# biomedia-mira/causal-gen

Hardware: AMD Instinct MI355X
Metric: HVAE train images/sec (higher is better)
Workload: dtype f16; 1 GPU; ukbb192 HVAE train step (192x192x1, DGauss likelihood, beta=5.0, z_max_res=96); per_gpu_batch=32, global_batch=32, parallelism=dp1, hipgraph=True, params=17371122

## Files before the change

causal-gen_amd/_lib.py:

```python
import ctypes as C
import os

_HERE = os.path.dirname(os.path.abspath(__file__))
LIB_PATH = os.environ.get("CGEN_LIB") or os.path.join(_HERE, "libcgen_hip.so")

F32, F16, F32S = 0, 1, 2
DMOL_LOW_BIT = 0x100
ACT_NONE, ACT_RELU, ACT_GELU = 0, 1, 2
UNARY_LEAKY_RELU, UNARY_CLAMP_MIN, UNARY_ADD = 3, 4, 5
MAX_SEG = 4


class View(C.Structure):
    _fields_ = [("p", C.c_void_p), ("sn", C.c_int64), ("sh", C.c_int64), ("sw", C.c_int64), ("c", C.c_int32),
                ("cpad", C.c_int32)]


NULL_VIEW = View(None, 0, 0, 0, 0, 0)


class ConvArgs(C.Structure):
    _fields_ = [("dtype", C.c_int32), ("n", C.c_int32), ("h", C.c_int32), ("w", C.c_int32), ("ks", C.c_int32),
                ("nseg", C.c_int32), ("act", C.c_int32), ("dact", C.c_int32), ("seg", View * MAX_SEG),
                ("weight", C.c_void_p), ("bias", C.c_void_p), ("out", View), ("aux", View), ("res1", View), ("res2", View),
                ("out_rem", C.c_int64), ("res1_rem", C.c_int64)]


class Block3Out(C.Structure):
    _fields_ = [("w", C.c_void_p), ("bias", C.c_void_p), ("out", View), ("aux", View), ("res1", View),
                ("out_rem", C.c_int64), ("res1_rem", C.c_int64)]


class Block3Args(C.Structure):
    _fields_ = [("dtype", C.c_int32), ("n", C.c_int32), ("h", C.c_int32), ("w", C.c_int32), ("nseg", C.c_int32),
                ("nout", C.c_int32), ("pre_act", C.c_int32), ("reserved", C.c_int32), ("seg", View * MAX_SEG),
                ("w_a", C.c_void_p), ("bias_a", C.c_void_p), ("mid", View), ("mid_aux", View), ("o", Block3Out * 2), ("w_a16", C.c_void_p)]


class Block4Args(C.Structure):
    _fields_ = [("dtype", C.c_int32), ("n", C.c_int32), ("h", C.c_int32), ("w", C.c_int32), ("nseg", C.c_int32),
                ("nout", C.c_int32), ("fwd", C.c_int32), ("b", C.c_int32), ("seg", View * MAX_SEG),
                ("wimg", C.c_void_p * 3), ("bias", C.c_void_p * 3), ("mid", View * 3), ("mid_aux", View * 3), ("o", Block3Out * 3)]


class WgradArgs(C.Structure):
    _fields_ = [("dtype", C.c_int32), ("n", C.c_int32), ("h", C.c_int32), ("w", C.c_int32), ("ks", C.c_int32),
                ("nseg", C.c_int32), ("act", C.c_int32), ("nsplit", C.c_int32), ("seg", View * MAX_SEG), ("gout", View),
                ("partial_w", C.c_void_p), ("partial_b", C.c_void_p)]


class WprepDesc(C.Structure):
# ... 267 lines not shown
```

causal-gen_amd/csrc/block.hip:

```cpp
#include <stddef.h>
#include <stdlib.h>

#include <algorithm>
#include <type_traits>

#include "common.h"

namespace cgen {

typedef float f32x16 __attribute__((ext_vector_type(16)));
typedef short s16x2v __attribute__((ext_vector_type(2)));

__device__ uint4 g_b3zero[4];

#define B3_TW 16
#define B3_HW 20
#define B3_MW 18
#define B3_XS 80
constexpr int b3_ndi(int th) { return ((th + 4) * B3_HW + 47) / 48; }
constexpr int b3_xbytes(int th) { return 4 * b3_ndi(th) * 12 * B3_XS + 64; }
constexpr int b3_nmp(int th) { return (th + 2) * B3_MW; }

struct BV3 { const char* p; int sn, sh, sw; };
struct B3Out {
// ... 5 lines not shown
};
struct B3P {
  int N, H, W, nseg, nch, b, nout, nksB;
  int tiles_x, tiles_y, ntiles, ctot8;
  int ns, wb_persist, scratch_off, bias_off;
  int tm_off, tm_bytes, pad1, pad2;
  Div32 d_tx, d_ty;
  BV3 seg[3];
  int seg_koff[4];
  int seg_c8[3];
  int small, s_rows, s_strips, s_nmb;
  int s_mid_off, s_kt_off, s_red_off, s_dbg, s_segk0[3], s_segg[3];
  Div32 s_dg1, s_dxw, s_dw, s_dstrips, s_dnb;
  int rows, r_rs, r_sx, r_sy, r_res_tile, r_pad;
  const char* wA16;
  const char* wA;
  const float* biasA;
  BV3 mid, mid_aux;
  B3Out o[2];
  unsigned long long* stamps;
};

__device__ __forceinline__ void b3_pin(h16x8& v) { asm volatile("" : "+v"(v)); }
__device__ __forceinline__ h16x8 b3_relu8(h16x8 v) {
  union { h16x8 h; s16x2v s[4]; } c;
  c.h = v;
#pragma unroll
  for (int e = 0; e < 4; ++e) c.s[e] = __builtin_elementwise_max(c.s[e], (s16x2v){0, 0});
  return c.h;
}
// ... 933 lines not shown
  constexpr size_t off_b = (sizeof(B3P) + alignof(B3P) - 1) / alignof(B3P) * alignof(B3P);
  const int koff = second ? (int)off_b : 0;
  typedef const B3P __attribute__((address_space(4)))* kp_ptr;
  const B3P& p = *(const B3P*)(kp_ptr)((const char __attribute__((address_space(4)))*)__builtin_amdgcn_kernarg_segment_ptr() + koff);
  blk3s_body<false>(p, second ? (int)blockIdx.x - na : (int)blockIdx.x, second ? (int)gridDim.x - na : na, koff);
}

#define B3R_NW 8
#define B3R_XC 36
#define B3R_MC 34
#define B3R_NG 4
#define B3R_MR 16
constexpr int b3r_grpb(int nch) { return ((4 * B3R_XC * (nch * 4 + 1) * 16 + 1023) / 1024) * 1024; }
constexpr int b3r_mrowb(int nb) { return B3R_MC * ((nb & 1) ? nb : nb + 1) * 16; }
constexpr size_t b3r_lds(int nch, int nb) { return (size_t)B3R_NG * b3r_grpb(nch) + (size_t)B3R_MR * b3r_mrowb(nb) + 1024; }

template <bool PRE, int NCH, int NB, int RES>
__global__ __launch_bounds__(64 * B3R_NW, 2) void blk3r_kernel(B3P p) {
  __builtin_amdgcn_s_setprio(3);
  constexpr int G1 = NCH * 4 + 1, XS = G1 * 16, ROWB = B3R_XC * XS, GRPB = b3r_grpb(NCH), NINST = GRPB / 1024, IPW = (NINST + B3R_NW - 1) / B3R_NW;
  constexpr int NBS = (NB & 1) ? NB : NB + 1, MS = NBS * 16, MROWB = B3R_MC * MS;
  constexpr int KA = 9 * NCH, NKB = (9 * NB + 1) / 2;
  constexpr bool AUX = !PRE;
  typedef __attribute__((address_space(3))) void* lds_ptr;
  extern __shared__ __attribute__((aligned(16))) char smem[];
  char* const X = smem;
  char* const MID = smem + B3R_NG * GRPB;
  char* const SCR = MID + B3R_MR * MROWB;
  const char* const zero = (const char*)g_b3zero;
  const int tid = threadIdx.x, lane = tid & 63, wave = __builtin_amdgcn_readfirstlane(tid >> 6);
  const int H = p.H, W = p.W, bch = p.b;
  const int item = blockIdx.x;
  const int sx = item % p.r_sx, t1 = item / p.r_sx, sy = t1 % p.r_sy, n = t1 / p.r_sy;
  const int x0 = sx * 32, Y0 = sy * p.r_rs, Yend = min(Y0 + p.r_rs, H), nbands = (Yend - Y0 + 3) >> 2;
  const BV3 sv = p.seg[0];
  const char* const xin = sv.p + n * sv.sn;
  auto dma_group = [&](const int gi) {
    const uint32_t gbase = (uint32_t)(uintptr_t)(lds_ptr)(X + (gi & (B3R_NG - 1)) * GRPB);
    const uint32_t sbase = (uint32_t)(uintptr_t)(lds_ptr)SCR;
    const int row0 = Y0 - 2 + 4 * gi;
#pragma unroll
    for (int t = 0; t < IPW; ++t) {
      const int ii = wave + B3R_NW * t;
      const int sl = ii * 64 + lane;
      const int r = sl / (B3R_XC * G1), rem = sl - r * (B3R_XC * G1), px = rem / G1, g = rem - px * G1;
      const int iy = row0 + r, ix = x0 - 2 + px;
      const bool ok = ii < NINST && r < 4 && (unsigned)iy < (unsigned)H && (unsigned)ix < (unsigned)W && g < G1 - 1;
      const char* src = ok ? xin + iy * sv.sh + ix * sv.sw + g * 16 : zero;
      b3_dma16(src, ii < NINST ? gbase + ii * 1024 : sbase);
    }
  };
  dma_group(0);
  dma_group(1);
  dma_group(2);
  h16x8 Aw[KA], Bw[NKB];
  {
    const char* wa = p.wA16 + lane * 16;
#pragma unroll
    for (int s_ = 0; s_ < KA; ++s_) Aw[s_] = *(const h16x8*)(wa + s_ * 1024);
    const int pair_w = min(wave >> 2, p.o[0].npb - 1);
    const char* wb = p.o[0].w + (size_t)pair_w * NKB * 1024 + lane * 16;
#pragma unroll
    for (int i = 0; i < NKB; ++i) Bw[i] = *(const h16x8*)(wb + i * 1024);
  }
  const int l16 = lane & 15, l4 = lane >> 4;
  int pr[2], pc[2];
#pragma unroll
  for (int j = 0; j < 2; ++j) {
    const int q = min(16 * (wave + B3R_NW * j) + l16, 4 * B3R_MC - 1);
    pr[j] = q / B3R_MC; pc[j] = q - pr[j] * B3R_MC;
  }
  const int chA = 4 * l4;
  float biasA[4] = {0.f, 0.f, 0.f, 0.f};
  if constexpr (PRE) {
    if (p.biasA != nullptr && chA < bch) { const float4 b4 = *(const float4*)(p.biasA + chA); biasA[0] = b4.x; biasA[1] = b4.y; biasA[2] = b4.z; biasA[3] = b4.w; }
  }
  const B3Out& O = p.o[0];
  const int npb = O.npb, Co = O.Co;
  const int pairB = wave >> 2, rB = wave & 3;
  const bool jobB = pairB < npb;
  const int pxB = lane & 31, kgB = lane >> 5;
  const int ch0 = pairB * 32 + 16 * kgB;
  int koff[NKB], kty[NKB];
#pragma unroll
  for (int i = 0; i < NKB; ++i) {
    const int u = 2 * i + kgB, tp = min(u / NB, 8), gq = u - (u / NB) * NB;
    kty[i] = tp / 3;
    koff[i] = (pxB + tp % 3) * MS + gq * 16;
  }
  float biasB[16];
#pragma unroll
  for (int e = 0; e < 16; ++e) biasB[e] = 0.f;
  if (jobB && O.bias != nullptr) {
#pragma unroll
    for (int e = 0; e < 16; e += 4)
      if (ch0 + e < Co) { const float4 b4 = *(const float4*)(O.bias + ch0 + e); biasB[e] = b4.x; biasB[e + 1] = b4.y; biasB[e + 2] = b4.z; biasB[e + 3] = b4.w; }
  }
  B3_VMWAIT();
#pragma unroll
  for (int s_ = 0; s_ < KA; ++s_) b3_pin(Aw[s_]);
#pragma unroll
  for (int i = 0; i < NKB; ++i) b3_pin(Bw[i]);
#pragma unroll
  for (int e = 0; e < 4; ++e) asm volatile("" : "+v"(biasA[e]));
#pragma unroll
  for (int e = 0; e < 16; ++e) asm volatile("" : "+v"(biasB[e]));
  B3_BARRIER();

  b3_u32x2 tm[2];
  b3_u32x4 ea[2], er[2];
  tm[0] = tm[1] = (b3_u32x2){0u, 0u};
  ea[0] = ea[1] = er[0] = er[1] = (b3_u32x4){0u, 0u, 0u, 0u};
  auto band_loads = [&](const int m0, const int nrow, const int y) {
    if constexpr (!PRE) {
#pragma unroll
      for (int j = 0; j < 2; ++j) {
        const int m = m0 + pr[j], col = x0 - 1 + pc[j];
        const bool ok = 16 * (wave + B3R_NW * j) + l16 < nrow * B3R_MC && (unsigned)m < (unsigned)H && (unsigned)col < (unsigned)W && chA < bch;
        b3_gload_v8(tm[j], ok ? p.mid_aux.p + (n * p.mid_aux.sn + m * p.mid_aux.sh + col * p.mid_aux.sw) + chA * 2 : zero);
      }
    }
// ... 56 lines not shown
        r.s[0] = __builtin_elementwise_max(r.s[0], (s16x2v){0, 0});
        r.s[1] = __builtin_elementwise_max(r.s[1], (s16x2v){0, 0});
        ol = r.u;
      } else {
        v[0] = h_lo(tm[j].x) > 0.f ? v[0] : 0.f; v[1] = h_hi(tm[j].x) > 0.f ? v[1] : 0.f;
        v[2] = h_lo(tm[j].y) > 0.f ? v[2] : 0.f; v[3] = h_hi(tm[j].y) > 0.f ? v[3] : 0.f;
        o.x = f2h_pk(v[0], v[1]); o.y = f2h_pk(v[2], v[3]);
        ol = o;
      }
      if (own) *(uint2*)((char*)p.mid.p + (n * p.mid.sn + m * p.mid.sh + col * p.mid.sw) + chA * 2) = o;
      *(uint2*)(MID + (m & (B3R_MR - 1)) * MROWB + pc[j] * MS + chA * 2) = in_img ? ol : make_uint2(0, 0);
    }
  };
  band_loads(Y0 - 1, 2, -1);
  phaseA(Y0 - 1, 2, 0);
  for (int k = 0; k < nbands; ++k) {
    const int Y = Y0 + 4 * k, y = Y + rB;
    B3_BARRIER();
    band_loads(Y + 1, 4, y);
    dma_group(k + 3);
    phaseA(Y + 1, 4, 1);
    B3_BARRIER();
    if (jobB) {
      const int ox = x0 + pxB;
      const bool ev = y < Yend && ox < W;
      int rowb[3];
#pragma unroll
      for (int ty = 0; ty < 3; ++ty) rowb[ty] = ((y - 1 + ty) & (B3R_MR - 1)) * MROWB;
      f32x16 c;
#pragma unroll
      for (int e = 0; e < 16; ++e) c[e] = biasB[e];
#pragma unroll
      for (int i = 0; i < NKB; ++i) {
        const int rb = kty[i] == 0 ? rowb[0] : (kty[i] == 1 ? rowb[1] : rowb[2]);
        const h16x8 bq = *(const h16x8*)(MID + rb + koff[i]);
        c = b3_mfma(Bw[i], bq, c);
      }
      if constexpr (RES == 1) {
        const int rel = y - (Y0 - 2);
        const char* rp = X + ((rel >> 2) & (B3R_NG - 1)) * GRPB + (rel & 3) * ROWB + (pxB + 2) * XS + (ch0 >> 3) * 16;
        er[0] = *(const b3_u32x4*)rp;
        er[1] = *(const b3_u32x4*)(rp + 16);
      }
#pragma unroll
      for (int q8 = 0; q8 < 2; ++q8) {
        if (!(ev && ch0 + 8 * q8 < Co)) continue;
        float u[8];
#pragma unroll
        for (int e = 0; e < 8; ++e) u[e] = c[8 * q8 + e];
        if constexpr (AUX) {
          const uint32_t w[4] = {ea[q8].x, ea[q8].y, ea[q8].z, ea[q8].w};
#pragma unroll
          for (int e = 0; e < 4; ++e) {
            u[2 * e] = h_lo(w[e]) > 0.f ? u[2 * e] : 0.f;
            u[2 * e + 1] = h_hi(w[e]) > 0.f ? u[2 * e + 1] : 0.f;
          }
        }
        if constexpr (RES != 0) {
          const uint32_t w[4] = {er[q8].x, er[q8].y, er[q8].z, er[q8].w};
#pragma unroll
          for (int e = 0; e < 4; ++e) { u[2 * e] += h_lo(w[e]); u[2 * e + 1] += h_hi(w[e]); }
        }
        *(uint4*)((char*)O.out.p + (n * O.out.sn + y * O.out.sh + ox * O.out.sw) + ch0 * 2 + 16 * q8) = b3_pack8(u);
      }
    }
  }
  B3_VMWAIT();
}

static bool b3_view(const cgen_view& v, int n, int h, int w, BV3& o) {
  o.p = (const char*)v.p; o.sn = o.sh = o.sw = 0;
  if (!v.p) return true;
  const int64_t ext = ((int64_t)n * v.sn + (int64_t)(h + 12 + 4) * v.sh + (int64_t)(w + B3_TW + 4) * v.sw + v.c + 64) * 2;
  if (ext >= ((int64_t)1 << 31) || v.sn < 0 || v.sh < 0 || v.sw < 0) return false;
  if (((uintptr_t)v.p % 16) || (v.sn * 2) % 16 || (v.sh * 2) % 16 || (v.sw * 2) % 16) return false;
  o.sn = (int)(v.sn * 2); o.sh = (int)(v.sh * 2); o.sw = (int)(v.sw * 2);
  return true;
}
// ... 40 lines not shown
    if (s.out_rem < 0 || s.res1_rem < 0 || s.out_rem >= ((int64_t)1 << 31) || s.res1_rem >= ((int64_t)1 << 31) || (s.out_rem % 16) || (s.res1_rem % 16)) return 0;
    if ((s.out_rem || s.res1_rem) && (!a->pre_act || a->nout != 1)) return 0;
    if (s.res1_rem && !s.res1.p) return 0;
    d.out_rem = (int)s.out_rem; d.res_rem = (int)s.res1_rem;
    if (!b3_view(s.out, a->n, a->h, a->w, d.out) || !b3_view(s.aux, a->n, a->h, a->w, d.aux) || !b3_view(s.res1, a->n, a->h, a->w, d.res)) return 0;
    if ((s.aux.p && s.aux.c != s.out.c) || (s.res1.p && s.res1.c != s.out.c)) return 0;
    if (o == 0 && s.out.c > 224 && !p.small) return 0;
    if (o > 0 && s.bias) return 0;
  }
  {
    static const int rows_on = [] { const char* e = getenv("CGEN_BLK3R"); return e ? atoi(e) : 1; }();
    const int c0 = a->seg[0].c, co0 = a->o[0].out.c;
    p.rows = (rows_on && !p.small && a->w_a16 && a->nseg == 1 && a->nout == 1 && (c0 == 32 || c0 == 64) && (p.b == 8 || p.b == 16)
              && (co0 == 32 || co0 == 64) && a->w >= 48 && a->h >= 16 && !a->o[0].out_rem && !a->o[0].res1_rem
              && ((uintptr_t)a->w_a16 % 16) == 0) ? 1 : 0;
    if (p.rows) {
      p.wA16 = (const char*)a->w_a16;
      p.r_sx = ceil_div(p.W, 32);
      const int slots = 256;
      long best = -1;
      for (int rs = 8; rs < p.H + 4; rs += 4) {
        const int rsc = rs > p.H ? ((p.H + 3) & ~3) : rs;
        const long wgs = (long)p.N * p.r_sx * ceil_div(p.H, rsc), cost = (long)ceil_div(wgs, slots) * (rsc + 16);
        if (best < 0 || cost < best) { best = cost; p.r_rs = rsc; }
      }
      { static const int rs_env = [] { const char* e = getenv("CGEN_BLK3R_RS"); return e ? atoi(e) : 0; }(); if (rs_env >= 4) p.r_rs = std::min((rs_env + 3) & ~3, (p.H + 3) & ~3); }
      p.r_sy = ceil_div(p.H, p.r_rs);
      p.ntiles = p.N * p.r_sx * p.r_sy;
      const cgen_view& rv = a->o[0].res1;
      p.r_res_tile = (a->pre_act && rv.p && rv.p == a->seg[0].p && rv.sn == a->seg[0].sn && rv.sh == a->seg[0].sh && rv.sw == a->seg[0].sw && co0 == c0) ? 1 : 0;
// ... 131 lines not shown
  if (pa.rows || pb.rows) return 0;
  if (pa.small || pb.small) {
    La.grid = pa.ntiles; Lb.grid = pb.ntiles;
    La.lds = b3s_lds(pa); Lb.lds = b3s_lds(pb);
    La.npg = Lb.npg = 0; La.sm = Lb.sm = 0; La.th = Lb.th = 0;
    return (pa.small && pb.small && !pa.o[0].out_rem && !pb.o[0].out_rem) ? 1 : 0;
  }
  const int ta = pa.ntiles, tb = pb.ntiles;
  La = b3_plan(pa, tb);
  Lb = b3_plan(pb, ta);
  if (La.sm || Lb.sm || La.npg != Lb.npg || La.th != Lb.th || pa.b != pb.b) return 0;
  if (pa.o[0].out_rem || pa.o[0].res_rem || pb.o[0].out_rem || pb.o[0].res_rem) return 0;
  return 1;
}

}

using namespace cgen;

extern "C" int cgen_block3_pair_supported(const cgen_block3_args* a, const cgen_block3_args* b) {
  B3P pa, pb;
  B3Launch La, Lb;
  return b3_pair_plan(a, b, pa, pb, La, Lb);
}

extern "C" int cgen_block3_pair(const cgen_block3_args* a, const cgen_block3_args* b, cgen_stream_t stream) {
  B3P pa, pb;
  B3Launch La, Lb;
  CGEN_REQUIRE(b3_pair_plan(a, b, pa, pb, La, Lb), "cgen_block3_pair: the two problems do not plan to the same data-gradient instance (ask cgen_block3_pair_supported first)");
  if (pa.small) {
// ... 11 lines not shown
  if (trace) fprintf(stderr, "blk3 pair[bwd] %dx%dx%d b %d | grids %d + %d, lds %zu, tile rows %d\n", a->n, a->h, a->w, pa.b, La.grid, Lb.grid, std::max(La.lds, Lb.lds), La.th);
  return check_launch("cgen_block3_pair");
}

extern "C" int cgen_block3_supported(const cgen_block3_args* a) {
  B3P p;
  return b3_fill(a, p);
}

extern "C" int cgen_block3(const cgen_block3_args* a, cgen_stream_t stream) {
  B3P p;
  CGEN_REQUIRE(b3_fill(a, p), "cgen_block3: shape / layout not served by the fused Block kernel (ask cgen_block3_supported first)");
  CGEN_REQUIRE((a->pre_act != 0) == (a->mid_aux.p == nullptr), "cgen_block3: pre_act = 1 is the forward pass (no mid_aux), pre_act = 0 the data gradient (mid_aux = the forward mid)");
  if (p.rows) {
    const int nch = a->seg[0].c / 32, nb = p.b / 8;
    const size_t lds = b3r_lds(nch, nb);
#define B3R_LAUNCH(PRE_, NCH_, NB_, RES_) do { (void)hipFuncSetAttribute((const void*)blk3r_kernel<PRE_, NCH_, NB_, RES_>, hipFuncAttributeMaxDynamicSharedMemorySize, 160 * 1024); \
    hipLaunchKernelGGL((blk3r_kernel<PRE_, NCH_, NB_, RES_>), dim3(p.ntiles), dim3(64 * B3R_NW), lds, (hipStream_t)stream, p); } while (0)
#define B3R_RES(PRE_, NCH_, NB_) do { if (res_mode == 0) B3R_LAUNCH(PRE_, NCH_, NB_, 0); else if (res_mode == 1) B3R_LAUNCH(PRE_, NCH_, NB_, 1); else B3R_LAUNCH(PRE_, NCH_, NB_, 2); } while (0)
#define B3R_RES_BWD(NCH_, NB_) do { if (res_mode == 0) B3R_LAUNCH(false, NCH_, NB_, 0); else B3R_LAUNCH(false, NCH_, NB_, 2); } while (0)
    const int res_mode = !a->o[0].res1.p ? 0 : (p.r_res_tile ? 1 : 2);
    if (a->pre_act) { if (nch == 1) { if (nb == 1) B3R_RES(true, 1, 1); else B3R_RES(true, 1, 2); } else { if (nb == 1) B3R_RES(true, 2, 1); else B3R_RES(true, 2, 2); } }
    else { if (nch == 1) { if (nb == 1) B3R_RES_BWD(1, 1); else B3R_RES_BWD(1, 2); } else { if (nb == 1) B3R_RES_BWD(2, 1); else B3R_RES_BWD(2, 2); } }
#undef B3R_RES
#undef B3R_RES_BWD
#undef B3R_LAUNCH
    static const bool trace_r = getenv("CGEN_CONV_TRACE") != nullptr;
    if (trace_r) fprintf(stderr, "blk3r[%s] %dx%dx%d c %d b %d Co %d | strips %d x %d of %d rows, grid %d, lds %zu, residual from the tile %d\n", a->mid_aux.p ? "bwd" : "fwd", a->n, a->h, a->w,
                         a->seg[0].c, p.b, p.o[0].Co, p.r_sx, p.r_sy, p.r_rs, p.ntiles, lds, p.r_res_tile);
    return check_launch("cgen_block3(rows)");
  }
  if (p.small) {
    const size_t lds = b3s_lds(p);
    if (a->pre_act) {
      (void)hipFuncSetAttribute((const void*)blk3s_kernel<true>, hipFuncAttributeMaxDynamicSharedMemorySize, 160 * 1024);
      hipLaunchKernelGGL((blk3s_kernel<true>), dim3(p.ntiles), dim3(64 * B3S_NW), lds, (hipStream_t)stream, p);
    } else {
      (void)hipFuncSetAttribute((const void*)blk3s_kernel<false>, hipFuncAttributeMaxDynamicSharedMemorySize, 160 * 1024);
// ... 14 lines not shown
```

causal-gen_amd/engine.py:

```python
import ctypes as C
import os
import math

import torch

from . import _lib
from .pairing import BlockRec, PairSlot, may_pair
from .wgrad_sched import WgradMixin
from ._lib import ACT_GELU, ACT_NONE, ACT_RELU, F16, F32, F32S, NULL_VIEW, UNARY_CLAMP_MIN, UNARY_LEAKY_RELU, View

_ALIGN = 256


def _ceil(a, m):
    return (a + m - 1) // m * m


def compact_parents(t):
    if t.dim() == 2:
        return t
    if t.dim() == 4 and ((t.shape[2] == 1 and t.shape[3] == 1) or (t.stride(2) == 0 and t.stride(3) == 0)):
        return t[:, :, 0, 0]
    return None

# ... 251 lines not shown
        self._wg_deferred = []
        self.fwd_branch = os.environ.get("CGEN_FWD_BRANCH", "1") != "0"
        self.infer_branch = os.environ.get("CGEN_INFER_BRANCH", "1") != "0"
        self.fwd_mainfirst = os.environ.get("CGEN_FWD_MAINFIRST", "1") != "0"
        self._fwd_side = None
        self._side_join_pending = False
        self.blk3_on = int(os.environ.get("CGEN_BLK3", "2")) if self.dt == F16 else 0
        self.blk3_minres = int(os.environ.get("CGEN_BLK3_MINRES", "16"))
        self.blk3_small = int(os.environ.get("CGEN_BLK3S", "1"))
        self.blk4_on = int(os.environ.get("CGEN_BLK4", "1")) if self.dt == F16 else 0
        self.blk4_launches = 0
        self.blk4_pair = os.environ.get("CGEN_BLK4_PAIR", "1") != "0"
        self._blk4 = PairSlot(self, self._block4_single, self._block4_pair,
                              lambda h, a: self.lib.block4_pair_supported(C.byref(h), C.byref(a)))
        self.blk3_rows = int(os.environ.get("CGEN_BLK3R", "1"))
        self.blk3_res = self._side_ranges(os.environ.get("CGEN_BLK3_RES", "20-64"))
        self.blk3_res3 = self._side_ranges(os.environ.get("CGEN_BLK3_RES3", "20-112"))
        self.split_frac = float(os.environ.get("CGEN_DP_SPLIT_FRAC", "0.8"))
        self.on_split = None
        self.early_final = None

    blk3_pairs = property(lambda self: self._blk3.pairs, lambda self, v: setattr(self._blk3, "pairs", v))
    blk4_pairs = property(lambda self: self._blk4.pairs, lambda self, v: setattr(self._blk4, "pairs", v))
    conv_pairs = property(lambda self: self._conv.pairs, lambda self, v: setattr(self._conv, "pairs", v))

    @property
    def trunk_rem(self):
        return self.dt != F32 and (self.trunk_mode >= 2 or (self.trunk_mode == 1 and not self.recording))

    def set_loss_scale(self, n_terms):
# ... 301 lines not shown
                self._dbg_names[id(out.base)] = site.name
            (self.tape if tape_hold is None else tape_hold).append((self._bw_conv, (site, segs, act, out, res1, res2), self._bw_tag))
        return out

    @staticmethod
    def _side_ranges(spec):
        out = []
        for v in spec.split(","):
            v = v.strip()
            if not v or v == "0":
                continue
            lo, _, hi = v.partition("-")
            out.append((int(lo), int(hi or lo)))
        return out

    def block2(self, site1, site2, segs, act, res1=None, trunk=False):
        x0 = segs[0]
        res_ok = self.blk3_res3 if len(segs) >= 3 else self.blk3_res
        small = self.blk3_small and x0.w <= 14 and x0.h <= 64 and min(x0.h, x0.w) >= 4
        tile_ok = (min(x0.h, x0.w) >= self.blk3_minres and site1.co <= 32
                   and (not res_ok or any(lo <= x0.h <= hi for lo, hi in res_ok)))
        rows = (self.blk3_rows and len(segs) == 1 and "a16_fwd" in site1.frag and "a16_dg" in site2.frag and x0.w >= 48 and x0.h >= 16
                and not (trunk and self.trunk_rem))
        if (self.blk3_on and act == ACT_RELU and "a_fwd" in site1.frag and "b_fwd" in site2.frag and len(segs) <= 3
                and site1.co % 8 == 0 and site2.co % 8 == 0
                and ((small and site1.co <= 64) or tile_ok or rows)):
            out = self._block3_fwd(site1, site2, segs, res1, trunk, need_rows=rows and not tile_ok and not small)
            if out is not None:
                return out
        t = self.conv(site1, segs, act)
        return self.conv(site2, [t], act, res1=res1, trunk=trunk)

# ... 16 lines not shown
        sup = self.lib.block3_supported(C.byref(a))
        if not sup or (need_rows and sup != 2):
            return None
        if not self._ablated(x0):
            self._timed("conv_fwd", (site1, site2), x0, lambda: self.lib.block3(C.byref(a), self.stream))
        if self.recording:
            if self._dbg_names is not None:
                self._dbg_names[id(out.base)] = site2.name
            if self.blk3_on >= 2:
                self.tape.append((self._bw_block3, BlockRec((site1, site2), segs, (t,), out, res1), self._bw_tag))
            else:
                self.tape.append((self._bw_conv, (site1, segs, ACT_RELU, t, None, None), self._bw_tag))
                self.tape.append((self._bw_conv, (site2, [t], ACT_RELU, out, res1, None), self._bw_tag))
        return out

    def _ablated(self, x0, site=None, tag=None):
        ab = self._ablate
        if not ab:
            return False
        if site is not None and ((tag in ab and site.name.endswith({"f1": ".conv.1", "d3": ".conv.3"}[tag])) or ("r12" in ab and x0.h <= 12)):
            return True
        return any(x0.h == r and ("r%d" % r) in ab for r in (24, 48, 96, 192))

    def _block3_dgrad_args(self, site1, site2, g, gmid, t, outs):
        a = _lib.Block3Args()
        a.dtype, a.n, a.h, a.w, a.nseg, a.nout, a.pre_act = self.dt, g.n, g.h, g.w, 1, len(outs), 0
        a.seg[0] = g.cv()
        a.w_a, a.bias_a = site2.frag["a_dg"], None
        a.w_a16 = site2.frag.get("a16_dg") if self.blk3_rows else None
        a.mid, a.mid_aux = gmid.cv(), t.cv()
        for j, (k, gv, sg, prev) in enumerate(outs):
            a.o[j].w, a.o[j].bias = site1.frag[("b_dg", k)], None
            a.o[j].out, a.o[j].aux = gv.cv(), sg.cv()
            a.o[j].res1 = prev.cv() if prev is not None else NULL_VIEW
        return a

    def _bw_block3(self, sites, segs, mids, out, res1):
        (site1, site2), (t,) = sites, mids
        g = self.grad_read(out)
        if g is None:
            self._blk3.flush()
            return
        act = ACT_RELU
        dsegs = [k for k, sg in enumerate(segs) if sg.rg and site1.seg_rg[k]]
        ok = (1 <= len(dsegs) <= 2 and "a_dg" in site2.frag and all(("b_dg", k) in site1.frag for k in dsegs)
              and all(segs[k].c % 8 == 0 for k in dsegs) and g.c % 8 == 0)
        if ok:
            probe = self._block3_dgrad_args(site1, site2, g, t, t, [(k, segs[k], segs[k], None) for k in dsegs])
            ok = bool(self.lib.block3_supported(C.byref(probe)))
        if not ok:
            self._blk3.flush()
            self._bw_conv(site2, [t], act, out, res1, None)
            self._bw_conv(site1, segs, act, t, None, None)
            return
        if res1 is not None and res1.rg:
            self._blk3.flush()
            self._grad_residual(res1, g, out, [t])
        if self._needs_wgrad(site2) and "wg" not in self._ablate:
            self._wgrad(site2, [t], act, g)
        gt, acc_t = self.grad_write(t)
        assert not acc_t
        tgt = [(k,) + self._dgrad_target(segs[k]) for k in dsegs]
        a = self._block3_dgrad_args(site1, site2, g, gt, t, [(k, gv, segs[k], prev if acc else None) for (k, gv, prev, acc) in tgt])
        x0 = segs[0]
        late = (lambda: self._wgrad(site1, segs, act, gt)) if (self._needs_wgrad(site1) and "wg" not in self._ablate) else (lambda: None)
        if self._ablated(x0):
            self._blk3.flush()
        elif self.lib.block3_supported(C.byref(a)):
            wr = {id(gt.base)} | {id(gv.base) for (_, gv, _, _) in tgt}
            rd = {id(g.base), id(t.base)} | {id(segs[k].base) for (k, _, _, _) in tgt} | {id(prev.base) for (_, _, prev, acc) in tgt if acc}
            self._blk3.submit(a, wr, rd, (sites, x0), late)
            return
        else:
            self._blk3.flush()
            self._dgrad_launch(site2, g, t, 0, act, t, gt, gt, False)
            for (k, gv, prev, acc) in tgt:
                self._dgrad_launch(site1, gt, segs[k], k, act, x0, gv, prev, acc)
        late()

    def _block3_single(self, a, info):
        sites, x0 = info
        self._timed("conv_dgrad", sites, x0, lambda: self.lib.block3(C.byref(a), self.stream))

    def block4(self, sites, segs, res1=None, trunk=False):
        s0, s1, s2, s3 = sites
# ... 550 lines not shown
            self._wg_total = sum(2.0 * st.ci * st.taps * st.co * x0.n * x0.h * x0.w
                                 for fn, a, _ in self.tape for st, x0 in self._entry_sites(fn, a) if self._needs_wgrad(st))
        main_t = torch.cuda.current_stream(self.device)
        if self._side_join_pending:
            self.join_side()
        self.blk3_pairs = self.conv_pairs = self.blk4_pairs = self.lat_tails = 0
        skip = 0
        tape = self.tape
        for i in range(len(tape) - 1, -1, -1):
            fn, args, _ = tape[i]
            if fn == self._bw_block3 or fn == self._bw_block4:
                slot, other, on = (self._blk3, self._blk4, self.blk3_pair) if fn == self._bw_block3 else (self._blk4, self._blk3, self.blk4_pair)
                other.flush()
                if on and slot.held is None and may_pair(tape[i], tape[i - 1] if i > 0 else None):
                    slot.arm()
                fn(*args)
                slot.disarm()
            else:
                self._blk3.flush()
                self._blk4.flush()
                if skip:
                    skip -= 1
                    continue
                if self.lat_tail and fn == self._bw_conv and self.dt == F16 and self.prof is None:
                    ents = self._latent_tail_at(i)
                    if ents is not None and self._bw_latent_tail(*ents):
                        skip = (2 if ents[0] is not None else 1)
                        continue
                if self.conv_pair and fn == self._bw_conv and self.dt != F32 and self._two_unfused_blocks(i):
                    self._conv.arm()
                    fn(*args)
# ... 259 lines not shown
```

causal-gen_amd/vae.py:

```python
import math
import os
from typing import Dict, List, Optional

import numpy as np
import weakref

import torch
from torch import Tensor, nn

from . import _lib
from ._lib import ACT_GELU, ACT_NONE, ACT_RELU, NULL_VIEW
from .engine import ConvSite, Engine

EPS = -9


def _flat_f32(name, *ts):
    lib = _lib.load()
    _lib.require_gpu()
    out = []
    shape, dev = ts[0].shape, ts[0].device
    for t in ts:
        if not (isinstance(t, torch.Tensor) and t.is_cuda and t.device == dev and t.shape == shape):
            raise _lib.CgenError(f"{name}: expects same-shaped tensors on one GPU (there is no CPU path)")
# ... 67 lines not shown
        else:
            _block_sites(sites, n + ".prior", b.prior, [w], [True])
        if b.stochastic:
            _block_sites(sites, n + ".posterior", b.posterior, [w, ctx, w], [True, False, True])
        sites.append(ConvSite(n + ".z_proj", b.z_proj, [zd, ctx], [True, False], len(sites)))
        if not b.q_correction:
            sites.append(ConvSite(n + ".z_feat_proj", b.z_feat_proj, [zd, w], [True, True], len(sites)))
        _block_sites(sites, n + ".conv", b.conv, [w], [True])


def run_block(eng, blk, segs):
    site = lambda conv: eng.site_by_id[id(conv)]
    act = ACT_RELU if blk.light else ACT_GELU
    cs = blk.convs()
    res = None
    if blk.residual:
        x = segs[0]
        if x.c != cs[-1].out_channels:
            res = eng.conv(site(blk.width_proj), segs, ACT_NONE)
        else:
            res = x
    if blk.light and len(cs) == 2:
        h = eng.block2(site(cs[0]), site(cs[1]), segs, act, res1=res, trunk=blk.residual)
    else:
        h = None
        if not blk.light and len(cs) == 4 and site(cs[0]).blk4 is not None:
            h = eng.block4([site(c) for c in cs], segs, res1=res, trunk=blk.residual)
        if h is None:
            h = eng.conv(site(cs[0]), segs, act, res1=res if len(cs) == 1 else None, trunk=blk.residual and len(cs) == 1)
            for j, c in enumerate(cs[1:]):
# ... 1008 lines not shown
```

include/cgen_hip.h:

```cpp
#ifndef CGEN_HIP_H
#define CGEN_HIP_H

#include <stddef.h>
#include <stdint.h>

#ifdef __cplusplus
extern "C" {
#endif

typedef void* cgen_stream_t;

enum cgen_status { CGEN_OK = 0, CGEN_EINVAL = -1, CGEN_ELAUNCH = -2, CGEN_EUNSUPPORTED = -3 };
enum cgen_dtype { CGEN_F32 = 0, CGEN_F16 = 1,
                  CGEN_F32S = 2 };
enum cgen_act { CGEN_ACT_NONE = 0, CGEN_ACT_RELU = 1, CGEN_ACT_GELU = 2 };

typedef struct cgen_view {
  void* p;
  int64_t sn, sh, sw;
  int32_t c;
  int32_t cpad;
} cgen_view;

#define CGEN_MAX_SEG 4
// ... 18 lines not shown

typedef struct cgen_block3_out {
  const void* w;
  const float* bias;
  cgen_view out, aux, res1;
  int64_t out_rem, res1_rem;
} cgen_block3_out;
typedef struct cgen_block3_args {
  int32_t dtype, n, h, w, nseg, nout, pre_act, reserved;
  cgen_view seg[CGEN_MAX_SEG];
  const void* w_a;
  const float* bias_a;
  cgen_view mid, mid_aux;
  cgen_block3_out o[2];
  const void* w_a16;
} cgen_block3_args;
int cgen_block3_supported(const cgen_block3_args* a);
int cgen_block3(const cgen_block3_args* a, cgen_stream_t stream);
int cgen_block3_pair_supported(const cgen_block3_args* a, const cgen_block3_args* b);
int cgen_block3_pair(const cgen_block3_args* a, const cgen_block3_args* b, cgen_stream_t stream);

typedef struct cgen_block4_args {
  int32_t dtype, n, h, w, nseg, nout, fwd, b;
  cgen_view seg[CGEN_MAX_SEG];
  const void* wimg[3];
  const float* bias[3];
  cgen_view mid[3], mid_aux[3];
  cgen_block3_out o[3];
} cgen_block4_args;
int cgen_block4_supported(const cgen_block4_args* a);
// ... 387 lines not shown
```

Baseline: 2460 images/s.

## Fuse 1x1 width projection and 2x2 avg-pool into row-streamed block3 kernel

For light residual down-sampling blocks, the forward pass now computes the 1x1 width projection, adds it to the block output and average-pools 2x2 inside the blk3r kernel, writing only the pooled tensor. Separate projection-conv and pool launches and the full-resolution output round trip through memory go away. Backward folds the projection data-gradient into the block3 dgrad kernel and skips the following tape entry. This costs extra LDS for a per-wave projection tile and a pooling exchange buffer, plus more registers, which may lower occupancy. The tape-skip bookkeeping also adds correctness risk.

```diff
diff --git a/causal-gen_amd/_lib.py b/causal-gen_amd/_lib.py
--- a/causal-gen_amd/_lib.py
+++ b/causal-gen_amd/_lib.py
@@ -34,7 +34,8 @@
 class Block3Args(C.Structure):
     _fields_ = [("dtype", C.c_int32), ("n", C.c_int32), ("h", C.c_int32), ("w", C.c_int32), ("nseg", C.c_int32),
                 ("nout", C.c_int32), ("pre_act", C.c_int32), ("reserved", C.c_int32), ("seg", View * MAX_SEG),
-                ("w_a", C.c_void_p), ("bias_a", C.c_void_p), ("mid", View), ("mid_aux", View), ("o", Block3Out * 2), ("w_a16", C.c_void_p)]
+                ("w_a", C.c_void_p), ("bias_a", C.c_void_p), ("mid", View), ("mid_aux", View), ("o", Block3Out * 2), ("w_a16", C.c_void_p),
+                ("w_proj", C.c_void_p), ("bias_proj", C.c_void_p), ("proj_krow", C.c_int32), ("pool", C.c_int32)]
 
 
 class Block4Args(C.Structure):
diff --git a/causal-gen_amd/csrc/block.hip b/causal-gen_amd/csrc/block.hip
--- a/causal-gen_amd/csrc/block.hip
+++ b/causal-gen_amd/csrc/block.hip
@@ -43,6 +43,9 @@
   Div32 s_dg1, s_dxw, s_dw, s_dstrips, s_dnb;
   int rows, r_rs, r_sx, r_sy, r_res_tile, r_pad;
   const char* wA16;
+  const char* wP;
+  const float* biasP;
+  int r_pkrow, r_pool;
   const char* wA;
   const float* biasA;
   BV3 mid, mid_aux;
@@ -1006,19 +1009,28 @@
 constexpr int b3r_grpb(int nch) { return ((4 * B3R_XC * (nch * 4 + 1) * 16 + 1023) / 1024) * 1024; }
 constexpr int b3r_mrowb(int nb) { return B3R_MC * ((nb & 1) ? nb : nb + 1) * 16; }
 constexpr size_t b3r_lds(int nch, int nb) { return (size_t)B3R_NG * b3r_grpb(nch) + (size_t)B3R_MR * b3r_mrowb(nb) + 1024; }
-
-template <bool PRE, int NCH, int NB, int RES>
+#define B3R_PJTS 144
+#define B3R_PJTB (32 * B3R_PJTS)
+constexpr size_t b3r_exb(int co) { return (size_t)4 * 32 * (co * 2 + 16); }
+
+template <bool PRE, int NCH, int NB, int RES, bool PROJ = false, int NR = 1>
 __global__ __launch_bounds__(64 * B3R_NW, 2) void blk3r_kernel(B3P p) {
   __builtin_amdgcn_s_setprio(3);
   constexpr int G1 = NCH * 4 + 1, XS = G1 * 16, ROWB = B3R_XC * XS, GRPB = b3r_grpb(NCH), NINST = GRPB / 1024, IPW = (NINST + B3R_NW - 1) / B3R_NW;
   constexpr int NBS = (NB & 1) ? NB : NB + 1, MS = NBS * 16, MROWB = B3R_MC * MS;
   constexpr int KA = 9 * NCH, NKB = (9 * NB + 1) / 2;
   constexpr bool AUX = !PRE;
+  constexpr bool POOL = PRE && PROJ;
+  constexpr int NKP = PROJ ? NCH : 1;
+  static_assert(!(PROJ && RES == 1) && !(POOL && RES != 0), "the projection replaces the residual");
+  static_assert(NR == 1 || POOL, "a second phase-B round exists for the pooled forward form only (no per-band epilogue loads)");
   typedef __attribute__((address_space(3))) void* lds_ptr;
   extern __shared__ __attribute__((aligned(16))) char smem[];
   char* const X = smem;
   char* const MID = smem + B3R_NG * GRPB;
   char* const SCR = MID + B3R_MR * MROWB;
+  char* const PJT = SCR + 1024;
+  char* const EXB = PJT + B3R_NW * B3R_PJTB;
   const char* const zero = (const char*)g_b3zero;
   const int tid = threadIdx.x, lane = tid & 63, wave = __builtin_amdgcn_readfirstlane(tid >> 6);
   const int H = p.H, W = p.W, bch = p.b;
@@ -1045,15 +1057,26 @@
   dma_group(0);
   dma_group(1);
   dma_group(2);
-  h16x8 Aw[KA], Bw[NKB];
+  h16x8 Aw[KA], Bw[NR][NKB], Pw[NR][2][NKP];
   {
     const char* wa = p.wA16 + lane * 16;
 #pragma unroll
     for (int s_ = 0; s_ < KA; ++s_) Aw[s_] = *(const h16x8*)(wa + s_ * 1024);
-    const int pair_w = min(wave >> 2, p.o[0].npb - 1);
+#pragma unroll
+    for (int r = 0; r < NR; ++r) {
+    const int pair_w = min((wave >> 2) + 2 * r, p.o[0].npb - 1);
     const char* wb = p.o[0].w + (size_t)pair_w * NKB * 1024 + lane * 16;
 #pragma unroll
-    for (int i = 0; i < NKB; ++i) Bw[i] = *(const h16x8*)(wb + i * 1024);
+    for (int i = 0; i < NKB; ++i) Bw[r][i] = *(const h16x8*)(wb + i * 1024);
+    if constexpr (PROJ) {
+#pragma unroll
+      for (int mt = 0; mt < 2; ++mt) {
+        const char* wp = p.wP + ((size_t)(pair_w * 32 + 16 * mt + (lane & 15)) * p.r_pkrow + 8 * (lane >> 4)) * 2;
+#pragma unroll
+        for (int i = 0; i < NKP; ++i) Pw[r][mt][i] = *(const h16x8*)(wp + i * 64);
+      }
+    }
+    }
   }
   const int l16 = lane & 15, l4 = lane >> 4;
   int pr[2], pc[2];
@@ -1080,23 +1103,48 @@
     kty[i] = tp / 3;
     koff[i] = (pxB + tp % 3) * MS + gq * 16;
   }
-  float biasB[16];
-#pragma unroll
-  for (int e = 0; e < 16; ++e) biasB[e] = 0.f;
-  if (jobB && O.bias != nullptr) {
-#pragma unroll
-    for (int e = 0; e < 16; e += 4)
-      if (ch0 + e < Co) { const float4 b4 = *(const float4*)(O.bias + ch0 + e); biasB[e] = b4.x; biasB[e + 1] = b4.y; biasB[e + 2] = b4.z; biasB[e + 3] = b4.w; }
-  }
+  float biasB[NR][16];
+  f32x4_t biasP[NR][2];
+#pragma unroll
+  for (int r = 0; r < NR; ++r) {
+    const int pairR = pairB + 2 * r, ch0R = ch0 + 64 * r;
+#pragma unroll
+    for (int e = 0; e < 16; ++e) biasB[r][e] = 0.f;
+    if (pairR < npb && O.bias != nullptr) {
+#pragma unroll
+      for (int e = 0; e < 16; e += 4)
+        if (ch0R + e < Co) { const float4 b4 = *(const float4*)(O.bias + ch0R + e); biasB[r][e] = b4.x; biasB[r][e + 1] = b4.y; biasB[r][e + 2] = b4.z; biasB[r][e + 3] = b4.w; }
+    }
+    biasP[r][0] = biasP[r][1] = (f32x4_t){0.f, 0.f, 0.f, 0.f};
+    if constexpr (POOL) {
+      if (pairR < npb && p.biasP != nullptr) {
+#pragma unroll
+        for (int mt = 0; mt < 2; ++mt) { const float4 b4 = *(const float4*)(p.biasP + pairR * 32 + 16 * mt + 4 * l4); biasP[r][mt] = (f32x4_t){b4.x, b4.y, b4.z, b4.w}; }
+      }
+    }
+  }
+  const int exs = Co * 2 + 16;
+  const int pl_ng = Co >> 3, pl_pp = tid / pl_ng, pl_cg = tid - pl_pp * pl_ng, pl_px = pl_pp & 15, pl_r = pl_pp >> 4;
   B3_VMWAIT();
 #pragma unroll
   for (int s_ = 0; s_ < KA; ++s_) b3_pin(Aw[s_]);
 #pragma unroll
-  for (int i = 0; i < NKB; ++i) b3_pin(Bw[i]);
-#pragma unroll
   for (int e = 0; e < 4; ++e) asm volatile("" : "+v"(biasA[e]));
 #pragma unroll
-  for (int e = 0; e < 16; ++e) asm volatile("" : "+v"(biasB[e]));
+  for (int r = 0; r < NR; ++r) {
+#pragma unroll
+    for (int i = 0; i < NKB; ++i) b3_pin(Bw[r][i]);
+#pragma unroll
+    for (int e = 0; e < 16; ++e) asm volatile("" : "+v"(biasB[r][e]));
+    if constexpr (PROJ) {
+#pragma unroll
+      for (int mt = 0; mt < 2; ++mt) {
+#pragma unroll
+        for (int i = 0; i < NKP; ++i) b3_pin(Pw[r][mt][i]);
+        asm volatile("" : "+v"(biasP[r][mt]));
+      }
+    }
+  }
   B3_BARRIER();
 
   b3_u32x2 tm[2];
@@ -1183,6 +1231,7 @@
   };
   band_loads(Y0 - 1, 2, -1);
   phaseA(Y0 - 1, 2, 0);
+  const int ch0_ = ch0;
   for (int k = 0; k < nbands; ++k) {
     const int Y = Y0 + 4 * k, y = Y + rB;
     B3_BARRIER();
@@ -1190,7 +1239,10 @@
     dma_group(k + 3);
     phaseA(Y + 1, 4, 1);
     B3_BARRIER();
-    if (jobB) {
+#pragma unroll
+    for (int r = 0; r < NR; ++r) {
+      const int ch0 = ch0_ + 64 * r;
+      if (!(pairB + 2 * r < npb)) continue;
       const int ox = x0 + pxB;
       const bool ev = y < Yend && ox < W;
       int rowb[3];
@@ -1198,12 +1250,12 @@
       for (int ty = 0; ty < 3; ++ty) rowb[ty] = ((y - 1 + ty) & (B3R_MR - 1)) * MROWB;
       f32x16 c;
 #pragma unroll
-      for (int e = 0; e < 16; ++e) c[e] = biasB[e];
+      for (int e = 0; e < 16; ++e) c[e] = biasB[r][e];
 #pragma unroll
       for (int i = 0; i < NKB; ++i) {
         const int rb = kty[i] == 0 ? rowb[0] : (kty[i] == 1 ? rowb[1] : rowb[2]);
         const h16x8 bq = *(const h16x8*)(MID + rb + koff[i]);
-        c = b3_mfma(Bw[i], bq, c);
+        c = b3_mfma(Bw[r][i], bq, c);
       }
       if constexpr (RES == 1) {
         const int rel = y - (Y0 - 2);
@@ -1211,9 +1263,30 @@
         er[0] = *(const b3_u32x4*)rp;
         er[1] = *(const b3_u32x4*)(rp + 16);
       }
+      float cp[16];
+      if constexpr (PROJ) {
+        const int rel = y - (Y0 - 2);
+        const char* xq = X + ((rel >> 2) & (B3R_NG - 1)) * GRPB + (rel & 3) * ROWB + (l16 + 2) * XS + l4 * 16;
+        char* const tw = PJT + wave * B3R_PJTB;
+#pragma unroll
+        for (int nt = 0; nt < 2; ++nt)
+#pragma unroll
+          for (int mt = 0; mt < 2; ++mt) {
+            f32x4_t d = biasP[r][mt];
+#pragma unroll
+            for (int i = 0; i < NKP; ++i) d = mfma_h16(Pw[r][mt][i], *(const h16x8*)(xq + nt * 16 * XS + i * 64), d, 0, 0, 0);
+            *(f32x4_t*)(tw + (l16 + 16 * nt) * B3R_PJTS + (16 * mt + 4 * l4) * 4) = d;
+          }
+#pragma unroll
+        for (int q4 = 0; q4 < 4; ++q4) {
+          const f32x4_t d = *(const f32x4_t*)(tw + pxB * B3R_PJTS + (16 * kgB + 4 * q4) * 4);
+#pragma unroll
+          for (int e = 0; e < 4; ++e) cp[4 * q4 + e] = d[e];
+        }
+      }
 #pragma unroll
       for (int q8 = 0; q8 < 2; ++q8) {
-        if (!(ev && ch0 + 8 * q8 < Co)) continue;
+        if constexpr (!POOL) { if (!(ev && ch0 + 8 * q8 < Co)) continue; }
         float u[8];
 #pragma unroll
         for (int e = 0; e < 8; ++e) u[e] = c[8 * q8 + e];
@@ -1230,7 +1303,36 @@
 #pragma unroll
           for (int e = 0; e < 4; ++e) { u[2 * e] += h_lo(w[e]); u[2 * e + 1] += h_hi(w[e]); }
         }
-        *(uint4*)((char*)O.out.p + (n * O.out.sn + y * O.out.sh + ox * O.out.sw) + ch0 * 2 + 16 * q8) = b3_pack8(u);
+        if constexpr (PROJ) {
+          const uint4 rw = b3_pack8(PRE ? cp + 8 * q8 : u);
+          const uint32_t w[4] = {rw.x, rw.y, rw.z, rw.w};
+#pragma unroll
+          for (int e = 0; e < 4; ++e) {
+            if constexpr (PRE) { u[2 * e] += h_lo(w[e]); u[2 * e + 1] += h_hi(w[e]); }
+            else { u[2 * e] = h_lo(w[e]) + cp[8 * q8 + 2 * e]; u[2 * e + 1] = h_hi(w[e]) + cp[8 * q8 + 2 * e + 1]; }
+          }
+        }
+        if constexpr (POOL) *(uint4*)(EXB + (rB * 32 + pxB) * exs + ch0 * 2 + 16 * q8) = b3_pack8(u);
+        else *(uint4*)((char*)O.out.p + (n * O.out.sn + y * O.out.sh + ox * O.out.sw) + ch0 * 2 + 16 * q8) = b3_pack8(u);
+      }
+    }
+    if constexpr (POOL) {
+      B3_BARRIER();
+      if (pl_r < 2 && Y + 2 * pl_r + 1 < Yend && x0 + 2 * pl_px + 1 < W) {
+        const char* e0 = EXB + (2 * pl_r * 32 + 2 * pl_px) * exs + pl_cg * 16;
+        const uint4 v4[4] = {*(const uint4*)e0, *(const uint4*)(e0 + exs), *(const uint4*)(e0 + 32 * exs), *(const uint4*)(e0 + 33 * exs)};
+        float a8[8];
+#pragma unroll
+        for (int e = 0; e < 8; ++e) a8[e] = 0.f;
+#pragma unroll
+        for (int q = 0; q < 4; ++q) {
+          const uint32_t w[4] = {v4[q].x, v4[q].y, v4[q].z, v4[q].w};
+#pragma unroll
+          for (int e = 0; e < 4; ++e) { a8[2 * e] += h_lo(w[e]); a8[2 * e + 1] += h_hi(w[e]); }
+        }
+#pragma unroll
+        for (int e = 0; e < 8; ++e) a8[e] *= 0.25f;
+        *(uint4*)((char*)O.out.p + (n * O.out.sn + ((Y >> 1) + pl_r) * O.out.sh + ((x0 >> 1) + pl_px) * O.out.sw) + pl_cg * 16) = b3_pack8(a8);
       }
     }
   }
@@ -1301,6 +1403,15 @@
     p.rows = (rows_on && !p.small && a->w_a16 && a->nseg == 1 && a->nout == 1 && (c0 == 32 || c0 == 64) && (p.b == 8 || p.b == 16)
               && (co0 == 32 || co0 == 64) && a->w >= 48 && a->h >= 16 && !a->o[0].out_rem && !a->o[0].res1_rem
               && ((uintptr_t)a->w_a16 % 16) == 0) ? 1 : 0;
+    if (a->w_proj || a->bias_proj || a->proj_krow || a->pool) {
+      const bool fwd = a->pre_act != 0;
+      if (!p.rows || !a->w_proj || ((uintptr_t)a->w_proj % 16) || ((uintptr_t)a->bias_proj % 16) || a->proj_krow < c0 || a->proj_krow % 8) return 0;
+      if (fwd ? !(a->pool == 2 && a->h % 2 == 0 && a->w % 2 == 0 && !a->o[0].res1.p && !a->mid_aux.p)
+              : !(a->pool == 0 && !a->bias_proj && a->mid_aux.p)) return 0;
+      if (b3r_lds(c0 / 32, p.b / 8) + (size_t)B3R_NW * B3R_PJTB + (fwd ? b3r_exb(co0) : 0) > 160 * 1024) return 0;
+      if (fwd && !b3_view(a->o[0].out, a->n, a->h / 2, a->w / 2, p.o[0].out)) return 0;
+      p.wP = (const char*)a->w_proj; p.biasP = a->bias_proj; p.r_pkrow = a->proj_krow; p.r_pool = a->pool;
+    }
     if (p.rows) {
       p.wA16 = (const char*)a->w_a16;
       p.r_sx = ceil_div(p.W, 32);
@@ -1462,6 +1573,12 @@
   return 1;
 }
 
+#ifdef B3R_TRIAL
+template __global__ void blk3r_kernel<true, 2, 2, 0, true, 2>(B3P);
+template __global__ void blk3r_kernel<false, 3, 2, 0, true, 1>(B3P);
+template __global__ void blk3r_kernel<false, 3, 2, 2, true, 1>(B3P);
+#endif
+
 }
 
 using namespace cgen;
@@ -1503,14 +1620,18 @@
   CGEN_REQUIRE((a->pre_act != 0) == (a->mid_aux.p == nullptr), "cgen_block3: pre_act = 1 is the forward pass (no mid_aux), pre_act = 0 the data gradient (mid_aux = the forward mid)");
   if (p.rows) {
     const int nch = a->seg[0].c / 32, nb = p.b / 8;
-    const size_t lds = b3r_lds(nch, nb);
-#define B3R_LAUNCH(PRE_, NCH_, NB_, RES_) do { (void)hipFuncSetAttribute((const void*)blk3r_kernel<PRE_, NCH_, NB_, RES_>, hipFuncAttributeMaxDynamicSharedMemorySize, 160 * 1024); \
-    hipLaunchKernelGGL((blk3r_kernel<PRE_, NCH_, NB_, RES_>), dim3(p.ntiles), dim3(64 * B3R_NW), lds, (hipStream_t)stream, p); } while (0)
+    const size_t lds = b3r_lds(nch, nb) + (p.wP ? (size_t)B3R_NW * B3R_PJTB : 0) + (p.r_pool ? b3r_exb(p.o[0].Co) : 0);
+#define B3R_LAUNCH(PRE_, NCH_, NB_, RES_, ...) do { (void)hipFuncSetAttribute((const void*)blk3r_kernel<PRE_, NCH_, NB_, RES_, ##__VA_ARGS__>, hipFuncAttributeMaxDynamicSharedMemorySize, 160 * 1024); \
+    hipLaunchKernelGGL((blk3r_kernel<PRE_, NCH_, NB_, RES_, ##__VA_ARGS__>), dim3(p.ntiles), dim3(64 * B3R_NW), lds, (hipStream_t)stream, p); } while (0)
 #define B3R_RES(PRE_, NCH_, NB_) do { if (res_mode == 0) B3R_LAUNCH(PRE_, NCH_, NB_, 0); else if (res_mode == 1) B3R_LAUNCH(PRE_, NCH_, NB_, 1); else B3R_LAUNCH(PRE_, NCH_, NB_, 2); } while (0)
 #define B3R_RES_BWD(NCH_, NB_) do { if (res_mode == 0) B3R_LAUNCH(false, NCH_, NB_, 0); else B3R_LAUNCH(false, NCH_, NB_, 2); } while (0)
     const int res_mode = !a->o[0].res1.p ? 0 : (p.r_res_tile ? 1 : 2);
-    if (a->pre_act) { if (nch == 1) { if (nb == 1) B3R_RES(true, 1, 1); else B3R_RES(true, 1, 2); } else { if (nb == 1) B3R_RES(true, 2, 1); else B3R_RES(true, 2, 2); } }
+#define B3R_DOWN(NCH_, NB_) do { if (a->pre_act) B3R_LAUNCH(true, NCH_, NB_, 0, true); else if (res_mode == 0) B3R_LAUNCH(false, NCH_, NB_, 0, true); else B3R_LAUNCH(false, NCH_, NB_, 2, true); } while (0)
+    if (p.wP) {
+      if (nch == 1) { if (nb == 1) B3R_DOWN(1, 1); else B3R_DOWN(1, 2); } else { if (nb == 1) B3R_DOWN(2, 1); else B3R_DOWN(2, 2); }
+    } else if (a->pre_act) { if (nch == 1) { if (nb == 1) B3R_RES(true, 1, 1); else B3R_RES(true, 1, 2); } else { if (nb == 1) B3R_RES(true, 2, 1); else B3R_RES(true, 2, 2); } }
     else { if (nch == 1) { if (nb == 1) B3R_RES_BWD(1, 1); else B3R_RES_BWD(1, 2); } else { if (nb == 1) B3R_RES_BWD(2, 1); else B3R_RES_BWD(2, 2); } }
+#undef B3R_DOWN
 #undef B3R_RES
 #undef B3R_RES_BWD
 #undef B3R_LAUNCH
diff --git a/causal-gen_amd/engine.py b/causal-gen_amd/engine.py
--- a/causal-gen_amd/engine.py
+++ b/causal-gen_amd/engine.py
@@ -289,6 +289,7 @@
         self._blk4 = PairSlot(self, self._block4_single, self._block4_pair,
                               lambda h, a: self.lib.block4_pair_supported(C.byref(h), C.byref(a)))
         self.blk3_rows = int(os.environ.get("CGEN_BLK3R", "1"))
+        self.blk3_down = int(os.environ.get("CGEN_BLK3_DOWN", "1")) if self.dt == F16 else 0
         self.blk3_res = self._side_ranges(os.environ.get("CGEN_BLK3_RES", "20-64"))
         self.blk3_res3 = self._side_ranges(os.environ.get("CGEN_BLK3_RES3", "20-112"))
         self.split_frac = float(os.environ.get("CGEN_DP_SPLIT_FRAC", "0.8"))
@@ -620,8 +621,10 @@
             out.append((int(lo), int(hi or lo)))
         return out
 
-    def block2(self, site1, site2, segs, act, res1=None, trunk=False):
+    def block2(self, site1, site2, segs, act, res1=None, trunk=False, proj=None, down=0):
         x0 = segs[0]
+        if proj is not None:
+            return self._block3_down_fwd(proj, site1, site2, segs, down)
         res_ok = self.blk3_res3 if len(segs) >= 3 else self.blk3_res
         small = self.blk3_small and x0.w <= 14 and x0.h <= 64 and min(x0.h, x0.w) >= 4
         tile_ok = (min(x0.h, x0.w) >= self.blk3_minres and site1.co <= 32
@@ -668,6 +671,58 @@
                 self.tape.append((self._bw_conv, (site2, [t], ACT_RELU, out, res1, None), self._bw_tag))
         return out
 
+    def _ghost(self, n, h, w, c):
+        cp = _ceil(c, 8)
+        return NT(0, n, h, w, c, h * w * cp, w * cp, cp, self.es)
+
+    def _block3_down_fwd(self, proj, site1, site2, segs, down):
+        x0 = segs[0]
+        if not (self.blk3_down and self.blk3_on and self.blk3_rows and len(segs) == 1 and isinstance(down, int) and down == 2
+                and proj.ks == 1 and proj.img_fwd is not None and "a_fwd" in site1.frag and "b_fwd" in site2.frag
+                and "a16_fwd" in site1.frag and x0.h % 2 == 0 and x0.w % 2 == 0):
+            return None
+        pc = proj.conv
+        assert (proj.ci == x0.c == site1.ci and proj.co == site2.co and tuple(pc.stride) == (1, 1) and tuple(pc.padding) == (0, 0)
+                and pc.groups == 1), (proj.name, "not a plain 1x1 projection of this Block's input onto its output width")
+        a = _lib.Block3Args()
+        a.dtype, a.n, a.h, a.w, a.nseg, a.nout, a.pre_act = self.dt, x0.n, x0.h, x0.w, 1, 1, 1
+        a.seg[0] = x0.cv()
+        b1, b2, bp = site1.conv.bias, site2.conv.bias, proj.conv.bias
+        a.w_a, a.bias_a = site1.frag["a_fwd"], (b1.data_ptr() if b1 is not None else None)
+        a.w_a16 = site1.frag["a16_fwd"]
+        a.w_proj, a.bias_proj, a.proj_krow, a.pool = proj.img_fwd, (bp.data_ptr() if bp is not None else None), proj.krow, 2
+        o = a.o[0]
+        o.w, o.bias = site2.frag["b_fwd"], (b2.data_ptr() if b2 is not None else None)
+        o.aux, o.res1 = NULL_VIEW, NULL_VIEW
+        def dense(h, w, c):
+            cp = _ceil(c, 8)
+            return View(x0.ptr, h * w * cp, w * cp, cp, c, 0)
+
+        a.mid, o.out = dense(x0.h, x0.w, site1.co), dense(x0.h // 2, x0.w // 2, site2.co)
+        if self.lib.block3_supported(C.byref(a)) != 2:
+            return None
+        t = self.new(x0.n, x0.h, x0.w, site1.co)
+        pooled = self.new(x0.n, x0.h // 2, x0.w // 2, site2.co)
+        a.mid, o.out = t.cv(), pooled.cv()
+        if self.lib.block3_supported(C.byref(a)) != 2:
+            raise RuntimeError("cgen_block3 declines the down Block's own tensors after serving the probe: %s" % (x0.shape,))
+        if not self._ablated(x0):
+            self._timed("conv_fwd", (proj, site1, site2), x0, lambda: self.lib.block3(C.byref(a), self.stream))
+        if self.recording:
+            res = self._ghost(x0.n, x0.h, x0.w, site2.co)
+            out = self._ghost(x0.n, x0.h, x0.w, site2.co)
+            if self._dbg_names is not None:
+                self._dbg_names[id(res.base)] = proj.name
+                self._dbg_names[id(out.base)] = site2.name
+            self.tape.append((self._bw_conv, (proj, segs, ACT_NONE, res, None, None), self._bw_tag))
+            if self.blk3_on >= 2:
+                self.tape.append((self._bw_block3, BlockRec((site1, site2), segs, (t,), out, res), self._bw_tag))
+            else:
+                self.tape.append((self._bw_conv, (site1, segs, ACT_RELU, t, None, None), self._bw_tag))
+                self.tape.append((self._bw_conv, (site2, [t], ACT_RELU, out, res, None), self._bw_tag))
+            self.tape.append((self._bw_pool, (out, pooled, down)))
+        return pooled
+
     def _ablated(self, x0, site=None, tag=None):
         ab = self._ablate
         if not ab:
@@ -676,8 +731,23 @@
             return True
         return any(x0.h == r and ("r%d" % r) in ab for r in (24, 48, 96, 192))
 
-    def _block3_dgrad_args(self, site1, site2, g, gmid, t, outs):
+    def _down_proj(self, segs, res1, blk_out, nbr):
+        prv, nxt = nbr if nbr is not None else (None, None)
+        if not (self.blk3_down and self.blk3_rows and nxt is not None and nxt[0] == self._bw_conv and res1 is not None and len(segs) == 1):
+            return None
+        if not (prv is not None and prv[0] == self._bw_pool and prv[1][0] is blk_out and isinstance(prv[1][2], int) and prv[1][2] == 2
+                and blk_out.h % 2 == 0 and blk_out.w % 2 == 0):
+            return None
+        site, psegs, act, out, r1, r2 = nxt[1]
+        ok = (site.ks == 1 and act == ACT_NONE and r1 is None and r2 is None and out is res1 and res1.base is res1 and res1.rg
+              and id(res1) not in self.grads and id(res1) not in self._riders and len(psegs) == 1 and psegs[0] is segs[0]
+              and segs[0].rg and site.seg_rg[0] and site.img_dg[0] is not None and not self._ablate)
+        return site if ok else None
+
+    def _block3_dgrad_args(self, site1, site2, g, gmid, t, outs, proj=None):
         a = _lib.Block3Args()
+        if proj is not None:
+            a.w_proj, a.proj_krow = proj.img_dg[0], proj.krow_dg
         a.dtype, a.n, a.h, a.w, a.nseg, a.nout, a.pre_act = self.dt, g.n, g.h, g.w, 1, len(outs), 0
         a.seg[0] = g.cv()
         a.w_a, a.bias_a = site2.frag["a_dg"], None
@@ -689,7 +759,7 @@
             a.o[j].res1 = prev.cv() if prev is not None else NULL_VIEW
         return a
 
-    def _bw_block3(self, sites, segs, mids, out, res1):
+    def _bw_block3(self, sites, segs, mids, out, res1, nbr=None):
         (site1, site2), (t,) = sites, mids
         g = self.grad_read(out)
         if g is None:
@@ -699,9 +769,14 @@
         dsegs = [k for k, sg in enumerate(segs) if sg.rg and site1.seg_rg[k]]
         ok = (1 <= len(dsegs) <= 2 and "a_dg" in site2.frag and all(("b_dg", k) in site1.frag for k in dsegs)
               and all(segs[k].c % 8 == 0 for k in dsegs) and g.c % 8 == 0)
+        proj = self._down_proj(segs, res1, out, nbr) if ok and len(dsegs) == 1 else None
         if ok:
-            probe = self._block3_dgrad_args(site1, site2, g, t, t, [(k, segs[k], segs[k], None) for k in dsegs])
+            probe = self._block3_dgrad_args(site1, site2, g, t, t, [(k, segs[k], segs[k], None) for k in dsegs], proj)
             ok = bool(self.lib.block3_supported(C.byref(probe)))
+            if not ok and proj is not None:
+                proj = None
+                probe = self._block3_dgrad_args(site1, site2, g, t, t, [(k, segs[k], segs[k], None) for k in dsegs])
+                ok = bool(self.lib.block3_supported(C.byref(probe)))
         if not ok:
             self._blk3.flush()
             self._bw_conv(site2, [t], act, out, res1, None)
@@ -715,7 +790,7 @@
         gt, acc_t = self.grad_write(t)
         assert not acc_t
         tgt = [(k,) + self._dgrad_target(segs[k]) for k in dsegs]
-        a = self._block3_dgrad_args(site1, site2, g, gt, t, [(k, gv, segs[k], prev if acc else None) for (k, gv, prev, acc) in tgt])
+        a = self._block3_dgrad_args(site1, site2, g, gt, t, [(k, gv, segs[k], prev if acc else None) for (k, gv, prev, acc) in tgt], proj)
         x0 = segs[0]
         late = (lambda: self._wgrad(site1, segs, act, gt)) if (self._needs_wgrad(site1) and "wg" not in self._ablate) else (lambda: None)
         if self._ablated(x0):
@@ -723,6 +798,16 @@
         elif self.lib.block3_supported(C.byref(a)):
             wr = {id(gt.base)} | {id(gv.base) for (_, gv, _, _) in tgt}
             rd = {id(g.base), id(t.base)} | {id(segs[k].base) for (k, _, _, _) in tgt} | {id(prev.base) for (_, _, prev, acc) in tgt if acc}
+            if proj is not None:
+                g_res, late1 = self.grad_read(res1), late
+
+                def late():
+                    late1()
+                    if self._needs_wgrad(proj) and "wg" not in self._ablate:
+                        self._wgrad(proj, segs, ACT_NONE, g_res)
+
+                self._blk3.submit(a, wr, rd, (sites + (proj,), x0), late)
+                return 1
             self._blk3.submit(a, wr, rd, (sites, x0), late)
             return
         else:
@@ -1303,7 +1388,10 @@
                 other.flush()
                 if on and slot.held is None and may_pair(tape[i], tape[i - 1] if i > 0 else None):
                     slot.arm()
-                fn(*args)
+                if fn == self._bw_block3:
+                    skip += fn(*args, nbr=(tape[i + 1] if i + 1 < len(tape) else None, tape[i - 1] if i > 0 else None)) or 0
+                else:
+                    fn(*args)
                 slot.disarm()
             else:
                 self._blk3.flush()
diff --git a/causal-gen_amd/vae.py b/causal-gen_amd/vae.py
--- a/causal-gen_amd/vae.py
+++ b/causal-gen_amd/vae.py
@@ -105,6 +105,10 @@
     act = ACT_RELU if blk.light else ACT_GELU
     cs = blk.convs()
     res = None
+    if blk.residual and blk.light and len(cs) == 2 and blk.d and segs[0].c != cs[-1].out_channels:
+        h = eng.block2(site(cs[0]), site(cs[1]), segs, act, trunk=True, proj=site(blk.width_proj), down=blk.d)
+        if h is not None:
+            return h
     if blk.residual:
         x = segs[0]
         if x.c != cs[-1].out_channels:
diff --git a/include/cgen_hip.h b/include/cgen_hip.h
--- a/include/cgen_hip.h
+++ b/include/cgen_hip.h
@@ -56,6 +56,9 @@
   cgen_view mid, mid_aux;
   cgen_block3_out o[2];
   const void* w_a16;
+  const void* w_proj;
+  const float* bias_proj;
+  int32_t proj_krow, pool;
 } cgen_block3_args;
 int cgen_block3_supported(const cgen_block3_args* a);
 int cgen_block3(const cgen_block3_args* a, cgen_stream_t stream);
```

Result: faster. 2485 images/s (median of 6 runs) (+1.0%).
